# facebookresearch/wmar

Hardware: AMD Instinct MI355X
Metric: watermarked images/sec at 256x256 (16x16 tok), batch 64; detector p-value delta vs ref (higher is better)
Workload: dtype f32; 1 GPU; Taming cin_transformer (48L x 1536d x 24h, V=16384) + VQGAN f16/16384, 256x256, batch 64 per GPU, greenlist watermark delta=2 gamma=0.25 h=1 (linear/stratifiedrand), T=1 top-k 250 top-p 0.92; sample -> decode -> re-encode -> detect; random-init weights; batch_per_gpu=64, decode_loop=hipGraph replay, backend=nccl

## Files before the change

include/wmar_hip.h:

```cpp
#ifndef WMAR_HIP_H
#define WMAR_HIP_H

#include <stdint.h>

#ifdef __cplusplus
extern "C" {
#endif

#define WMAR_OK 0
#define WMAR_EINVAL (-1)
#define WMAR_EHIP (-2)
#define WMAR_ESHORT (-3)
#define WMAR_MAX_CONTEXT 16
#define WMAR_ENOMEM (-4)
#define WMAR_EMISSING (-5)
#define WMAR_ECALLBACK (-6)

#define WMAR_SEED_FIXED 0
#define WMAR_SEED_LINEAR 1
#define WMAR_SEED_SPATIAL 2
#define WMAR_SPLIT_RAND 0
#define WMAR_SPLIT_STRATIFIED 1

const char* wmar_last_error(void);
// ... 206 lines not shown
int wmar_cham_sample(const wmar_wm_ctx* wm, const float* logits3_dev, int64_t B, int64_t V, const int64_t* past_ids_dev,
                     int64_t t, int64_t past_stride, float temperature, double top_p, float guidance_scale_text,
                     float guidance_scale_image, const uint32_t* allow_dev, const int32_t* allow_ids_dev, int32_t n_allow,
                     const float* q_dev, float* scratch_dev, int64_t* tok_out_dev, void* stream);

typedef struct wmar_vq_config {
    int32_t ch, num_res_blocks, resolution, in_channels, out_ch, z_channels, embed_dim, n_embed;
    int32_t n_levels;
    int32_t ch_mult[8];
    int32_t n_attn_res;
    int32_t attn_resolutions[8];
    int32_t max_batch;
} wmar_vq_config;

typedef struct wmar_vq wmar_vq;

int wmar_vq_create(const wmar_vq_config* cfg, const char* const* names, const void* const* tensors_dev,
                   int32_t n_tensors, void* stream, wmar_vq** out);
void wmar_vq_destroy(wmar_vq* v);
int64_t wmar_vq_device_bytes(const wmar_vq* v);

int wmar_vq_decode(wmar_vq* v, const int64_t* codes_dev, int64_t B, float* images_dev, void* stream);
int wmar_vq_encode(wmar_vq* v, const float* images_dev, int64_t B, int64_t* codes_dev, float* prequant_dev,
                   void* stream);

int wmar_vq_probe_conv(const float* w_dev, const float* bias_dev, int32_t cout, int32_t cin, int32_t ks, const float* x_dev,
                       const float* res_dev, const float* gn_gamma_dev, const float* gn_beta_dev, int32_t gn_swish, int64_t B, int32_t Hs,
                       int32_t Ws, int32_t stride, int32_t up, int32_t arm_stats, float* y_dev, float* out_mr_dev, char* kernel_buf,
                       int64_t buf_len, void* stream);
int wmar_vq_probe_attn(const float* q_dev, const float* k_dev, const float* v_dev, int64_t B, int32_t H, int32_t W, int32_t C, float* o_dev,
                       char* path_buf, int64_t buf_len, void* stream);
int wmar_vq_probe_argmin(const float* z_dev, int64_t P, int32_t E, const float* codebook_dev, int32_t n_embed, int64_t* codes_dev,
                         char* path_buf, int64_t buf_len, void* stream);

int wmar_vq_probe_conv_backward(const float* w_dev, int32_t cout, int32_t cin, int32_t ks, const float* x_dev, const float* gy_dev, int64_t B,
                                int32_t Hs, int32_t Ws, int32_t stride, int32_t up, float* gx_dev, float* gw_dev, float* gb_dev,
                                char* kernel_buf, int64_t buf_len, void* stream);
int wmar_vq_probe_gn_backward(const float* x_dev, const float* gy_dev, const float* mr_dev, const float* gamma_dev, const float* beta_dev,
                              int64_t B, int32_t HW, int32_t C, int32_t swish, float* gx_dev, float* dgamma_dev, float* dbeta_dev,
                              char* path_buf, int64_t buf_len, void* stream);
int wmar_vq_probe_attn_backward(const float* q_dev, const float* k_dev, const float* v_dev, const float* go_dev, int64_t B, int32_t H, int32_t W,
                                int32_t C, float* gq_dev, float* gk_dev, float* gv_dev, char* path_buf, int64_t buf_len, void* stream);

int wmar_vq_probe_avgpool_backward(const float* gy_dev, int64_t B, int32_t Ho, int32_t Wo, int32_t C, float* gx_dev, void* stream);
int wmar_mvq_probe_image_backward(const float* pre_dev, const float* g_nchw_dev, int64_t B, int32_t C, int32_t HW, int32_t Cs, float* g_nhwc_dev,
                                  void* stream);
int wmar_mvq_probe_input_backward(const float* g_nhwc_dev, int64_t B, int32_t C, int32_t HW, int32_t Cs, float* g_nchw_dev, void* stream);

typedef struct wmar_vq_train wmar_vq_train;
int wmar_vq_train_create(const wmar_vq_config* cfg, const char* const* names, const void* const* tensors_dev, int32_t n_tensors, void* stream,
                         wmar_vq_train** out);
void wmar_vq_train_destroy(wmar_vq_train* t);
int64_t wmar_vq_train_device_bytes(const wmar_vq_train* t);
int wmar_vq_train_set_weights(wmar_vq_train* t, const char* const* names, const void* const* tensors_dev, int32_t n_tensors, void* stream);
int wmar_vq_train_encode(wmar_vq_train* t, const float* images_dev, int64_t B, float* prequant_dev, void* stream);
int wmar_vq_train_encode_backward(wmar_vq_train* t, const float* grad_prequant_dev, int64_t B, float* grad_images_dev, void* stream);
int wmar_vq_train_decode(wmar_vq_train* t, const float* zq_dev, int64_t B, float* images_dev, void* stream);
int wmar_vq_train_decode_backward(wmar_vq_train* t, const float* grad_images_dev, int64_t B, float* grad_zq_dev, void* stream);
int wmar_vq_train_get_grads(wmar_vq_train* t, const char* const* names, void* const* grads_dev, int32_t n, int32_t accumulate, void* stream);

typedef struct wmar_mvq_config {
    int32_t hidden_channels, num_res_blocks, resolution, num_channels, z_channels, num_embeddings;
    int32_t n_levels;
    int32_t channel_mult[8];
    int32_t max_batch;
} wmar_mvq_config;
// ... 61 lines not shown
```

wmar_amd/_lib.py:

```python
from __future__ import annotations

import ctypes as C
import os

HERE = os.path.dirname(os.path.abspath(__file__))
LIB_PATH = os.path.join(HERE, "libwmar_hip.so")

SYMBOLS = [
    "wmar_last_error", "wmar_version", "wmar_key_row_words", "wmar_key_table_rows", "wmar_key_table_build",
    "wmar_key_greenlist", "wmar_wm_process_logits", "wmar_sample_fused", "wmar_detect", "wmar_detect_num_ngrams",
    "wmar_gpt_create", "wmar_gpt_destroy", "wmar_gpt_device_bytes", "wmar_gpt_decode_step", "wmar_gpt_generate",
    "wmar_gpt_set_timing", "wmar_gpt_set_attention_phases", "wmar_gpt_get_timing", "wmar_gpt_profile_role", "wmar_gpt_plan_info", "wmar_gpt_check",
    "wmar_gpt_probe_run", "wmar_gpt_probe_copy", "wmar_gpt_probe_plan", "wmar_rar_create", "wmar_rar_destroy",
    "wmar_rar_device_bytes", "wmar_rar_forward_position", "wmar_rar_generate", "wmar_vq_create", "wmar_vq_destroy", "wmar_vq_device_bytes",
    "wmar_vq_decode", "wmar_vq_encode", "wmar_vq_probe_conv", "wmar_vq_probe_attn", "wmar_vq_probe_argmin", "wmar_vq_probe_conv_backward", "wmar_vq_probe_gn_backward", "wmar_vq_probe_attn_backward",
    "wmar_vq_probe_avgpool_backward", "wmar_mvq_probe_image_backward", "wmar_mvq_probe_input_backward", "wmar_mvq_train_create",
    "wmar_vq_train_create", "wmar_vq_train_destroy", "wmar_vq_train_device_bytes", "wmar_vq_train_set_weights", "wmar_vq_train_encode",
    "wmar_vq_train_encode_backward", "wmar_vq_train_decode", "wmar_vq_train_decode_backward", "wmar_vq_train_get_grads", "wmar_mvq_create", "wmar_mvq_destroy", "wmar_mvq_device_bytes", "wmar_mvq_decode",
    "wmar_mvq_encode", "wmar_gumbel_key_build", "wmar_gumbel_sample", "wmar_gumbel_score", "wmar_gumbel_key_rows", "wmar_gumbel_score_ctx", "wmar_rar_generate_gumbel", "wmar_rar_generate_gumbel_ctx", "wmar_rar_check", "wmar_rar_launch_status",
    "wmar_cham_create", "wmar_cham_destroy", "wmar_cham_device_bytes", "wmar_cham_forward_tokens", "wmar_cham_generate_image",
    "wmar_cham_sample", "wmar_cham_probe_run", "wmar_cham_probe_copy", "wmar_cham_probe_plan",
    "wmar_cfg_mix", "wmar_gpt_generate_hooked", "wmar_rar_generate_hooked", "wmar_cham_generate_image_hooked",
    "wmar_augment", "wmar_augment_backward", "wmar_jpeg_workspace_bytes", "wmar_jpeg", "wmar_resample_coeffs", "wmar_image_ingest",
    "wmar_sync_positions", "wmar_sync_workspace_bytes", "wmar_sync_fit", "wmar_sync_rotate_labels",
    "wmar_comm_unique_id", "wmar_comm_init", "wmar_comm_bcast", "wmar_comm_allgather", "wmar_comm_rank", "wmar_comm_world", "wmar_comm_destroy",
]

WMAR_ESHORT = -3
WMAR_ECALLBACK = -6

LOGITS_HOOK = C.CFUNCTYPE(C.c_int, C.c_void_p, C.c_int32, C.c_int64)


class KeyParams(C.Structure):
    _fields_ = [("salt_key", C.c_uint64), ("alive_ids", C.POINTER(C.c_int64)), ("n_alive", C.c_int64),
                ("dead_ids", C.POINTER(C.c_int64)), ("n_dead", C.c_int64), ("vocab_size", C.c_int64),
                ("gamma", C.c_double), ("split_strategy", C.c_int32), ("seed_strategy", C.c_int32)]


class WmCtx(C.Structure):
    _fields_ = [("table_dev", C.c_void_p), ("n_rows", C.c_int64), ("vocab_size", C.c_int64),
                ("seed_strategy", C.c_int32), ("context_size", C.c_int32), ("spatial_dim", C.c_int32),
                ("delta", C.c_float)]


class GptConfig(C.Structure):
    _fields_ = [("vocab_size", C.c_int32), ("block_size", C.c_int32), ("n_layer", C.c_int32),
                ("n_head", C.c_int32), ("n_embd", C.c_int32), ("max_batch", C.c_int32)]
# ... 110 lines not shown
    L.wmar_gpt_plan_info.argtypes = [vp, i64, C.c_char_p, i64]
    L.wmar_gpt_check.argtypes = [vp, vp]
    L.wmar_gpt_probe_run.argtypes = [vp, vp, i64, i32, i32, i32, i32, vp, vp]
    L.wmar_gpt_probe_copy.restype = i64
    L.wmar_gpt_probe_copy.argtypes = [vp, C.c_char_p, i32, vp, i64, i32, vp]
    L.wmar_gpt_probe_plan.argtypes = [vp, i64, i32, C.c_char_p, i64]
    L.wmar_rar_create.argtypes = [C.POINTER(RarConfig), C.POINTER(C.c_char_p), C.POINTER(vp), i32, vp, C.POINTER(vp)]
    L.wmar_rar_destroy.argtypes = [vp]
    L.wmar_rar_destroy.restype = None
    L.wmar_rar_device_bytes.restype = i64
    L.wmar_rar_device_bytes.argtypes = [vp]
    L.wmar_rar_forward_position.argtypes = [vp, vp, vp, i64, i32, vp, vp]
    L.wmar_rar_generate.argtypes = [vp, C.POINTER(WmCtx), vp, i64, C.POINTER(f32), i32, f32, vp, vp, i32, vp]
    L.wmar_rar_generate_gumbel.argtypes = [vp, vp, i64, C.POINTER(f32), i32, f32, f32, i32, vp, vp, i32, vp]
    L.wmar_rar_generate_gumbel_ctx.argtypes = [vp, vp, i64, C.POINTER(f32), i32, f32, f32, i32, C.c_uint64, i32, vp, vp, i32, vp]
    L.wmar_rar_check.argtypes = [vp, vp]
    L.wmar_rar_launch_status.argtypes = [vp, C.POINTER(i32), C.POINTER(i32)]
    L.wmar_gumbel_key_build.argtypes = [C.c_uint64, i64, vp, vp, vp]
    L.wmar_gumbel_sample.argtypes = [vp, i64, i64, vp, i64, i32, f32, f32, i32, vp, vp]
    L.wmar_gumbel_score.argtypes = [vp, i64, i64, i64, vp, i64, vp, vp, vp]
    L.wmar_gumbel_key_rows.argtypes = [vp, i64, i64, vp, vp, vp, vp]
    L.wmar_gumbel_score_ctx.argtypes = [vp, i64, i64, i64, C.c_uint64, i32, vp, vp, vp, vp]
    if hasattr(L, "wmar_vq_create"):
        L.wmar_vq_create.argtypes = [C.POINTER(VqConfig), C.POINTER(C.c_char_p), C.POINTER(vp), i32, vp, C.POINTER(vp)]
        L.wmar_vq_destroy.argtypes = [vp]
        L.wmar_vq_destroy.restype = None
        L.wmar_vq_device_bytes.restype = i64
        L.wmar_vq_device_bytes.argtypes = [vp]
        L.wmar_vq_decode.argtypes = [vp, vp, i64, vp, vp]
        L.wmar_vq_encode.argtypes = [vp, vp, i64, vp, vp, vp]
        L.wmar_vq_probe_conv.argtypes = [vp, vp, i32, i32, i32, vp, vp, vp, vp, i32, i64, i32, i32, i32, i32, i32, vp, vp, C.c_char_p, i64, vp]
        L.wmar_vq_probe_attn.argtypes = [vp, vp, vp, i64, i32, i32, i32, vp, C.c_char_p, i64, vp]
        L.wmar_vq_probe_argmin.argtypes = [vp, i64, i32, vp, i32, vp, C.c_char_p, i64, vp]
        L.wmar_vq_probe_conv_backward.argtypes = [vp, i32, i32, i32, vp, vp, i64, i32, i32, i32, i32, vp, vp, vp, C.c_char_p, i64, vp]
        L.wmar_vq_probe_gn_backward.argtypes = [vp, vp, vp, vp, vp, i64, i32, i32, i32, vp, vp, vp, C.c_char_p, i64, vp]
        L.wmar_vq_probe_attn_backward.argtypes = [vp, vp, vp, vp, i64, i32, i32, i32, vp, vp, vp, C.c_char_p, i64, vp]
        L.wmar_vq_probe_avgpool_backward.argtypes = [vp, i64, i32, i32, i32, vp, vp]
        L.wmar_mvq_probe_image_backward.argtypes = [vp, vp, i64, i32, i32, i32, vp, vp]
        L.wmar_mvq_probe_input_backward.argtypes = [vp, i64, i32, i32, i32, vp, vp]
        L.wmar_mvq_train_create.argtypes = [C.POINTER(MvqConfig), C.POINTER(C.c_char_p), C.POINTER(vp), i32, vp, C.POINTER(vp)]
        L.wmar_vq_train_create.argtypes = [C.POINTER(VqConfig), C.POINTER(C.c_char_p), C.POINTER(vp), i32, vp, C.POINTER(vp)]
        L.wmar_vq_train_destroy.argtypes = [vp]
        L.wmar_vq_train_destroy.restype = None
        L.wmar_vq_train_device_bytes.restype = i64
        L.wmar_vq_train_device_bytes.argtypes = [vp]
        L.wmar_vq_train_set_weights.argtypes = [vp, C.POINTER(C.c_char_p), C.POINTER(vp), i32, vp]
        L.wmar_vq_train_encode.argtypes = [vp, vp, i64, vp, vp]
        L.wmar_vq_train_encode_backward.argtypes = [vp, vp, i64, vp, vp]
        L.wmar_vq_train_decode.argtypes = [vp, vp, i64, vp, vp]
        L.wmar_vq_train_decode_backward.argtypes = [vp, vp, i64, vp, vp]
        L.wmar_vq_train_get_grads.argtypes = [vp, C.POINTER(C.c_char_p), C.POINTER(vp), i32, i32, vp]
    L.wmar_cham_create.argtypes = [C.POINTER(ChamConfig), C.POINTER(C.c_char_p), C.POINTER(vp), i32, vp, C.POINTER(vp)]
    L.wmar_cham_destroy.argtypes = [vp]
    L.wmar_cham_destroy.restype = None
    L.wmar_cham_device_bytes.restype = i64
    L.wmar_cham_device_bytes.argtypes = [vp]
    L.wmar_cham_forward_tokens.argtypes = [vp, vp, vp, i64, vp, vp]
    L.wmar_cham_probe_run.argtypes = [vp, vp, vp, i64, i32, i32, i32, vp, vp]
    L.wmar_cham_probe_copy.restype = i64
    L.wmar_cham_probe_copy.argtypes = [vp, C.c_char_p, i32, vp, i64, i32, vp]
    L.wmar_cham_probe_plan.argtypes = [vp, i64, C.c_char_p, i64]
    L.wmar_cham_generate_image.argtypes = [vp, C.POINTER(WmCtx), vp, vp, i64, C.POINTER(ChamSampleParams), vp, vp, i32, vp, i32, vp, vp]
    L.wmar_cham_sample.argtypes = [C.POINTER(WmCtx), vp, i64, i64, vp, i64, i64, f32, f64, f32, f32, vp, vp, i32, vp, vp, vp, vp]
    L.wmar_cfg_mix.argtypes = [vp, vp, vp, vp, i64, i64, vp, vp, f32, f32, vp]
    L.wmar_gpt_generate_hooked.argtypes = [vp, C.POINTER(SampleParams), vp, i64, i32, vp, vp, vp, vp, i64, LOGITS_HOOK, vp, vp]
    L.wmar_rar_generate_hooked.argtypes = [vp, vp, i64, C.POINTER(f32), i32, f32, vp, vp, i32, vp, vp, i64, LOGITS_HOOK, vp, vp]
# ... 33 lines not shown
```

wmar_amd/csrc/vqgan.hip:

```cpp
#include <algorithm>
#include <map>
#include <memory>
#include <string>
#include <vector>

#include "common.h"
#include "bx_split.h"
#include "vq_plan.h"

namespace wmar {

using f32x16 = __attribute__((ext_vector_type(16))) float;

__global__ void k_pack_conv(const float* __restrict__ W, float4* __restrict__ Wp, int Cout, int Cin, int ks,
                            int CT, int KBc) {
    const int T = ks * ks;
    long long idx = (long long)blockIdx.x * blockDim.x + threadIdx.x;
    long long total = (long long)CT * T * KBc * 64;
    if (idx >= total) return;
    int lane = (int)(idx & 63);
    long long r = idx >> 6;
    int kb = (int)(r % KBc); r /= KBc;
    int tap = (int)(r % T);
    int ct = (int)(r / T);
// ... 7 lines not shown
    Wp[idx] = make_float4(v[0], v[1], v[2], v[3]);
}

__global__ void k_pack_conv_bx(const float* __restrict__ W, u32x4* __restrict__ Wq, int Cout, int Cin, int ks, int CT, int KU,
                               long long w_bstride = 0, long long wq_bstride = 0, int transposed = 0) {
    const int T = ks * ks;
    const long long idx = (long long)blockIdx.x * blockDim.x + threadIdx.x;
    if (idx >= (long long)CT * T * KU * 64) return;
    W += (long long)blockIdx.y * w_bstride;
    Wq += (long long)blockIdx.y * wq_bstride;
    const int lane = (int)(idx & 63);
    long long r = idx >> 6;
    const int ku = (int)(r % KU); r /= KU;
    const int tap = (int)(r % T);
    const int ct = (int)(r / T);
    const int co = ct * 32 + (lane & 31), ci0 = ku * 16 + 8 * (lane >> 5);
    float v[8];
    for (int i = 0; i < 8; ++i)
        v[i] = (co < Cout && ci0 + i < Cin) ? (transposed ? W[(long long)(ci0 + i) * Cout + co] : W[((long long)co * Cin + ci0 + i) * T + tap]) : 0.f;
    unsigned h[4], m[4], l[4];
    for (int i = 0; i < 4; ++i) bx_split2(v[2 * i], v[2 * i + 1], h[i], m[i], l[i]);
    u32x4* o = Wq + (idx >> 6) * 192 + lane;
    o[0] = u32x4{h[0], h[1], h[2], h[3]}; o[64] = u32x4{m[0], m[1], m[2], m[3]}; o[128] = u32x4{l[0], l[1], l[2], l[3]};
}

__global__ void k_pad_vec(const float* __restrict__ src, float* __restrict__ dst, int n, int npad) {
    int i = blockIdx.x * blockDim.x + threadIdx.x;
    if (i < npad) dst[i] = i < n ? src[i] : 0.f;
}

struct ConvArgs {
    const float* in;
    const float4* wp;
    const u32x4* wq;
    long long wq_bstride;
    const float* bias;
    const float* res;
    float* out;
    int Hs, Ws, Cin;
    int Ho, Wo, Cout_s;
    int CT, KBc;
    int ks, stride, up, pad;
    int tiles_x, tiles_y;
    int dbuf;
    const float2* gn_mr;
    const float* gn_g; const float* gn_b;
    int gn_cpg, gn_swish;
    double* st_part;
    int st_cpg;
};

__device__ __forceinline__ float4 conv_gn(const ConvArgs& a, float4 v, int b, int c) {
    const float4 g = *(const float4*)(a.gn_g + c), bt = *(const float4*)(a.gn_b + c);
    float r[4] = {v.x, v.y, v.z, v.w};
    const float gg[4] = {g.x, g.y, g.z, g.w}, bb[4] = {bt.x, bt.y, bt.z, bt.w};
    const float2* mr = a.gn_mr + b * 32;
    if (a.gn_cpg >= 4 && (a.gn_cpg & 3) == 0) {
        const float2 m = mr[c / a.gn_cpg];
#pragma unroll
        for (int i = 0; i < 4; ++i) r[i] = (r[i] - m.x) * m.y * gg[i] + bb[i];
    } else {
#pragma unroll
        for (int i = 0; i < 4; ++i) { const float2 m = mr[(c + i) / a.gn_cpg]; r[i] = (r[i] - m.x) * m.y * gg[i] + bb[i]; }
    }
    if (a.gn_swish)
#pragma unroll
        for (int i = 0; i < 4; ++i) r[i] = r[i] / (1.0f + __expf(-r[i]));
    return make_float4(r[0], r[1], r[2], r[3]);
}

__device__ __forceinline__ float4 conv_gn_apply(float4 v, const float4 g, const float4 bt, const float2 m, int swish) {
    float r[4] = {(v.x - m.x) * m.y * g.x + bt.x, (v.y - m.x) * m.y * g.y + bt.y, (v.z - m.x) * m.y * g.z + bt.z, (v.w - m.x) * m.y * g.w + bt.w};
    if (swish)
#pragma unroll
        for (int i = 0; i < 4; ++i) r[i] = r[i] / (1.0f + __expf(-r[i]));
    return make_float4(r[0], r[1], r[2], r[3]);
}

__device__ __forceinline__ void conv_store(const ConvArgs& a, const f32x16 (&acc)[2], int b, int ct, int ty, int tx, int lane) {
    const int j = lane & 31, half = lane >> 5;
    const int prow = j >> 3, pcol = j & 7;
    const int oy0 = ty * 8, ox0 = tx * 8;
    double gs[4] = {0.0, 0.0, 0.0, 0.0}, gss[4] = {0.0, 0.0, 0.0, 0.0};
#pragma unroll
    for (int p = 0; p < 2; ++p) {
        const int oy = oy0 + p * 4 + prow, ox = ox0 + pcol;
        const long long pix = ((long long)b * a.Ho + oy) * a.Wo + ox;
#pragma unroll
        for (int g = 0; g < 4; ++g) {
            const int co = ct * 32 + g * 8 + half * 4;
            if (co >= a.Cout_s) continue;
            const float4 bb = *(const float4*)(a.bias + co);
            float4 o = make_float4(acc[p][g * 4 + 0] + bb.x, acc[p][g * 4 + 1] + bb.y, acc[p][g * 4 + 2] + bb.z,
                                   acc[p][g * 4 + 3] + bb.w);
            if (a.res) {
                const float4 rr = *(const float4*)(a.res + pix * a.Cout_s + co);
                o.x += rr.x; o.y += rr.y; o.z += rr.z; o.w += rr.w;
            }
            *(float4*)(a.out + pix * a.Cout_s + co) = o;
            if (a.st_part) {
                gs[g] += (double)o.x + (double)o.y + (double)o.z + (double)o.w;
                gss[g] += sq4_f64(o);
            }
        }
    }
    if (a.st_part) {
        const int top = a.st_cpg >= 8 ? 32 : 16;
#pragma unroll
        for (int g = 0; g < 4; ++g)
            for (int o = 1; o <= top; o <<= 1) { gs[g] += __shfl_xor(gs[g], o); gss[g] += __shfl_xor(gss[g], o); }
        if (a.st_cpg == 16) { gs[0] += gs[1]; gss[0] += gss[1]; gs[2] += gs[3]; gss[2] += gss[3]; }
        const long long tile = ((long long)b * a.tiles_y + ty) * a.tiles_x + tx;
        double* dst = a.st_part + tile * 64;
        if (a.st_cpg == 4) {
            if ((lane & 31) == 0)
#pragma unroll
                for (int g = 0; g < 4; ++g) { const int grp = ct * 8 + 2 * g + half; dst[grp * 2] = gs[g]; dst[grp * 2 + 1] = gss[g]; }
        } else if (lane == 0) {
            if (a.st_cpg == 8) {
#pragma unroll
                for (int g = 0; g < 4; ++g) { const int grp = ct * 4 + g; dst[grp * 2] = gs[g]; dst[grp * 2 + 1] = gss[g]; }
            } else {
                dst[(ct * 2) * 2] = gs[0]; dst[(ct * 2) * 2 + 1] = gss[0];
                dst[(ct * 2 + 1) * 2] = gs[2]; dst[(ct * 2 + 1) * 2 + 1] = gss[2];
            }
        }
    }
}

constexpr int CONV_CCH = 32;
constexpr int CONV_PSTRIDE = 36;

template <int COT>
__global__ __launch_bounds__(COT * 64) void k_conv(ConvArgs a) {
    extern __shared__ __attribute__((aligned(16))) float patch[];
    const int lane = threadIdx.x & 63;
    const int w = __builtin_amdgcn_readfirstlane(threadIdx.x >> 6);
    int bid = blockIdx.x;
    const int tx = bid % a.tiles_x; bid /= a.tiles_x;
    const int ty = bid % a.tiles_y; bid /= a.tiles_y;
    const int cgroups = (a.CT + COT - 1) / COT;
    const int cg = bid % cgroups;
    const int b = bid / cgroups;
    const int ct = cg * COT + w;
    const bool active = ct < a.CT;
    const int T = a.ks * a.ks;
    const int PW = 7 * a.stride + a.ks, PH = PW;
    const int oy0 = ty * 8, ox0 = tx * 8;
    const int iy0 = oy0 * a.stride - a.pad, ix0 = ox0 * a.stride - a.pad;
    const int Hc = a.up ? a.Hs * 2 : a.Hs, Wc = a.up ? a.Ws * 2 : a.Ws;

    f32x16 acc[2];
#pragma unroll
    for (int i = 0; i < 2; ++i)
#pragma unroll
        for (int r = 0; r < 16; ++r) acc[i][r] = 0.f;

    const int j = lane & 31, half = lane >> 5;
    const int prow = j >> 3, pcol = j & 7;
    const float* inb = a.in + (long long)b * a.Hs * a.Ws * a.Cin;

#define WMAR_CONV_ROUND(PATCH, C0, CCH)                                                                         \
    if (active) {                                                                                               \
        const int nkb = (CCH) >> 3;                                                                             \
        const float4* wbase = a.wp + ((long long)ct * T * a.KBc + ((C0) >> 3)) * 64 + lane;                     \
        for (int tap = 0; tap < T; ++tap) {                                                                     \
            const int dy = tap / a.ks, dx = tap - dy * a.ks;                                                    \
            const float4* wt = wbase + (long long)tap * a.KBc * 64;                                             \
            const float* p0 = (PATCH) + (((prow)*a.stride + dy) * PW + pcol * a.stride + dx) * CONV_PSTRIDE + half * 4; \
            const float* p1 = p0 + 4 * a.stride * PW * CONV_PSTRIDE;                                            \
            _Pragma("unroll 4") for (int kb = 0; kb < nkb; ++kb) {                                              \
                const float4 wv = wt[kb * 64];                                                                  \
                const float4 x0 = *(const float4*)(p0 + kb * 8);                                                \
                const float4 x1 = *(const float4*)(p1 + kb * 8);                                                \
                acc[0] = __builtin_amdgcn_mfma_f32_32x32x2f32(wv.x, x0.x, acc[0], 0, 0, 0);                     \
                acc[1] = __builtin_amdgcn_mfma_f32_32x32x2f32(wv.x, x1.x, acc[1], 0, 0, 0);                     \
// ... 348 lines not shown
    if (threadIdx.x < 32) { acc[threadIdx.x][0] = 0; acc[threadIdx.x][1] = 0; }
    __syncthreads();
    __shared__ double tmp[256][4][2];
    for (int i = 0; i < 4; ++i) { tmp[threadIdx.x][i][0] = s[i]; tmp[threadIdx.x][i][1] = ss[i]; }
    __syncthreads();
    if (threadIdx.x < 32) {
        const int g = threadIdx.x;
        double ts = 0, tss = 0;
        for (int t = 0; t < 256; ++t) {
            if (t / q4 >= pstep) break;
            const int c = (t % q4) * 4;
            for (int i = 0; i < 4; ++i)
                if ((c + i) / cpg == g) { ts += tmp[t][i][0]; tss += tmp[t][i][1]; }
        }
        double* o = a.partial + (((long long)b * a.nchunk + chunk) * 32 + g) * 2;
        o[0] = ts; o[1] = tss;
    }
}

__global__ void k_gn_finalize(GnArgs a, float2* mr) {
    const int b = blockIdx.x, g = threadIdx.x;
    double ts = 0, tss = 0;
    for (int c = 0; c < a.nchunk; ++c) {
        const double* p = a.partial + (((long long)b * a.nchunk + c) * 32 + g) * 2;
        ts += p[0]; tss += p[1];
    }
    const double n = (double)a.HW * (a.C / 32);
    const double rn = inv_count_f64(n);
    const double mean = ts * rn;
    const double var = var_f64(tss * rn, mean);
    mr[b * 32 + g] = make_float2((float)mean, (float)rsqrt_f64(var + 1e-6));
}

__global__ __launch_bounds__(256) void k_gn_finalize_tiles(const double* part, int tiles, double count, float2* mr) {
    __shared__ double red[8][32][2];
    const int b = blockIdx.x, g = threadIdx.x & 31, q = threadIdx.x >> 5;
    const double* p = part + (long long)b * tiles * 64 + g * 2;
    double ts = 0, tss = 0;
    for (int t = q; t < tiles; t += 8) { ts += p[(long long)t * 64]; tss += p[(long long)t * 64 + 1]; }
    red[q][g][0] = ts; red[q][g][1] = tss;
    __syncthreads();
    if (threadIdx.x < 32) {
        ts = 0; tss = 0;
        for (int i = 0; i < 8; ++i) { ts += red[i][g][0]; tss += red[i][g][1]; }
        const double rn = inv_count_f64(count);
        const double mean = ts * rn;
        const double var = var_f64(tss * rn, mean);
        mr[b * 32 + g] = make_float2((float)mean, (float)rsqrt_f64(var + 1e-6));
    }
}

__global__ __launch_bounds__(256) void k_attn_scores(const float* __restrict__ q, const float* __restrict__ k,
                                                     float* __restrict__ sc, int N, int C, float scale) {
    extern __shared__ float qs[];
    __shared__ float red[4];
    const int b = blockIdx.y, i = blockIdx.x;
    const float* qi = q + ((long long)b * N + i) * C;
    for (int c = threadIdx.x; c < C; c += 256) qs[c] = qi[c];
    __syncthreads();
    float* row = sc + ((long long)b * N + i) * N;
    float mx = -INFINITY;
    for (int j = threadIdx.x; j < N; j += 256) {
        const float* kj = k + ((long long)b * N + j) * C;
        float s = 0.f;
        for (int c = 0; c < C; c += 4) {
            float4 kv = *(const float4*)(kj + c);
            s += qs[c] * kv.x + qs[c + 1] * kv.y + qs[c + 2] * kv.z + qs[c + 3] * kv.w;
        }
        s *= scale;
        row[j] = s;
        mx = fmaxf(mx, s);
    }
    for (int o = 32; o > 0; o >>= 1) mx = fmaxf(mx, __shfl_xor(mx, o));
    if ((threadIdx.x & 63) == 0) red[threadIdx.x >> 6] = mx;
    __syncthreads();
    mx = fmaxf(fmaxf(red[0], red[1]), fmaxf(red[2], red[3]));
    __syncthreads();
// ... 349 lines not shown
static thread_local int g_vq_splits = 0;

struct GnRef {
    const float2* mr; const float* g; const float* b; int C, swish;
};

int run_conv(const ConvW& c, const float* in, float* out, const float* res, int B, int Hs, int Ws, int stride, int up,
             hipStream_t st, const GnRef* gn = nullptr, long long wq_bstride = 0) {
    ConvArgs a{};
    if (gn) {
        WMAR_REQUIRE(gn->C == c.cin_s && !up, "fused GroupNorm: channel count %d != conv input %d", gn->C, c.cin_s);
        a.gn_mr = gn->mr; a.gn_g = gn->g; a.gn_b = gn->b; a.gn_cpg = gn->C / 32; a.gn_swish = gn->swish;
    }
    a.in = in; a.wp = c.wp; a.wq = c.wq; a.wq_bstride = wq_bstride; a.bias = c.bias; a.res = res; a.out = out;
    a.Hs = Hs; a.Ws = Ws; a.Cin = c.cin_s;
    const int Hc = up ? 2 * Hs : Hs, Wc = up ? 2 * Ws : Ws;
    a.Ho = stride == 2 ? Hc / 2 : Hc; a.Wo = stride == 2 ? Wc / 2 : Wc;
    a.Cout_s = c.cout_s; a.CT = c.CT; a.KBc = c.KBc; a.ks = c.ks; a.stride = stride; a.up = up;
    a.pad = (c.ks == 3 && stride == 1) ? 1 : 0;
    WMAR_REQUIRE(a.Ho % 8 == 0 && a.Wo % 8 == 0, "conv output %dx%d is not a multiple of the 8x8 tile", a.Ho, a.Wo);
    a.tiles_x = a.Wo / 8; a.tiles_y = a.Ho / 8;
    const int PW = 7 * stride + c.ks;
    const int COT = c.CT >= 4 ? 4 : (c.CT >= 2 ? 2 : 1);
    a.dbuf = (c.cin_s % CONV_CCH == 0 && PW * PW * 8 <= 4 * COT * 64) ? 1 : 0;
    const int cpg_out = c.cout / 32;
    const bool stats = wq_bstride == 0 && g_trk.part && c.cout == c.cout_s && c.cout % 32 == 0 && (cpg_out == 4 || cpg_out == 8 || cpg_out == 16) &&
                       (long long)B * a.tiles_x * a.tiles_y * 64 <= g_trk.cap;
    if (stats) { a.st_part = g_trk.part; a.st_cpg = cpg_out; g_trk.src = out; g_trk.tiles = a.tiles_x * a.tiles_y; g_trk.C = c.cout; }
    else if (g_trk.src == out) g_trk.src = nullptr;
    const bool bx2 = c.wq && c.cin_s % CONV_CCH == 0 && stride == 2 && c.ks == 3 && COT == 4 && !up && !conv_no_bx() && conv_s2_bx();
    const bool bx = (c.wq && c.cin_s % CONV_CCH == 0 && stride == 1 && (c.ks == 3 || c.ks == 1) && !conv_no_bx()) || bx2;
    if (bx) a.dbuf = 1;
    const bool wide = bx && !bx2 && COT == 4 && c.ks == 3 && a.tiles_x % 2 == 0 && wq_bstride == 0 && conv_pt4();
    const size_t lds = bx ? (size_t)2 * PW * (wide ? PW + 8 : PW) * CONV_PSTRIDE_BX : (size_t)(a.dbuf ? 2 : 1) * PW * PW * CONV_PSTRIDE * sizeof(float);
    const int cgroups = (c.CT + COT - 1) / COT;
    const unsigned grid = (unsigned)((long long)B * cgroups * (wide ? a.tiles_x / 2 : a.tiles_x) * a.tiles_y);
    hipEvent_t e0 = nullptr, e1 = nullptr;
    if (vq_trace()) { (void)hipEventCreate(&e0); (void)hipEventCreate(&e1); (void)hipEventRecord(e0, st); }
    static const bool few_off = getenv("WMAR_CONV_FEW_OFF") != nullptr;
    const bool few = c.wf && c.ks == 3 && stride == 1 && !up && !res && !stats && wq_bstride == 0 && c.cout <= 4 && a.Ho % CF_T == 0 &&
                     a.Wo % CF_T == 0 && !few_off;
    if (few) {
        a.tiles_x = a.Wo / CF_T; a.tiles_y = a.Ho / CF_T;
        const unsigned gridf = (unsigned)((long long)B * a.tiles_x * a.tiles_y);
        const size_t ldsf = (size_t)CF_PW * CF_PW * CONV_PSTRIDE * sizeof(float);
        if (c.cout == 3) { g_conv_kernel = "k_conv_few<3>"; hipLaunchKernelGGL(k_conv_few<3>, dim3(gridf), dim3(256), ldsf, st, a, (const float*)c.wf); }
        else { g_conv_kernel = "k_conv_few<4>"; hipLaunchKernelGGL(k_conv_few<4>, dim3(gridf), dim3(256), ldsf, st, a, (const float*)c.wf); }
    } else if (bx2) {
        static const hipError_t lds2_ok = hipFuncSetAttribute((const void*)k_conv_bx<4, 3, 2, 2>, hipFuncAttributeMaxDynamicSharedMemorySize, 160 * 1024);
        WMAR_REQUIRE(lds2_ok == hipSuccess, "k_conv_bx (stride 2): raising the dynamic LDS limit failed: %s", hipGetErrorString(lds2_ok));
        g_conv_kernel = "k_conv_bx<4,3,2,2>";
        hipLaunchKernelGGL((k_conv_bx<4, 3, 2, 2>), dim3(grid), dim3(256), lds, st, a);
    } else if (wide) {
        static const hipError_t lds_ok = hipFuncSetAttribute((const void*)k_conv_bx<4, 3, 4>, hipFuncAttributeMaxDynamicSharedMemorySize, 160 * 1024);
        WMAR_REQUIRE(lds_ok == hipSuccess, "k_conv_bx: raising the dynamic LDS limit failed: %s", hipGetErrorString(lds_ok));
        g_conv_kernel = "k_conv_bx<4,3,4>";
        hipLaunchKernelGGL((k_conv_bx<4, 3, 4>), dim3(grid), dim3(256), lds, st, a);
    }
    else if (bx && COT == 4 && c.ks == 3) { g_conv_kernel = "k_conv_bx<4,3>"; hipLaunchKernelGGL((k_conv_bx<4, 3>), dim3(grid), dim3(256), lds, st, a); }
    else if (bx && COT == 4) { g_conv_kernel = "k_conv_bx<4,1>"; hipLaunchKernelGGL((k_conv_bx<4, 1>), dim3(grid), dim3(256), lds, st, a); }
    else if (bx && COT == 2 && c.ks == 3) { g_conv_kernel = "k_conv_bx<2,3>"; hipLaunchKernelGGL((k_conv_bx<2, 3>), dim3(grid), dim3(128), lds, st, a); }
    else if (bx && COT == 2) { g_conv_kernel = "k_conv_bx<2,1>"; hipLaunchKernelGGL((k_conv_bx<2, 1>), dim3(grid), dim3(128), lds, st, a); }
    else if (bx && c.ks == 3) { g_conv_kernel = "k_conv_bx<1,3>"; hipLaunchKernelGGL((k_conv_bx<1, 3>), dim3(grid), dim3(64), lds, st, a); }
    else if (bx) { g_conv_kernel = "k_conv_bx<1,1>"; hipLaunchKernelGGL((k_conv_bx<1, 1>), dim3(grid), dim3(64), lds, st, a); }
    else if (COT == 4) { g_conv_kernel = "k_conv<4>"; hipLaunchKernelGGL(k_conv<4>, dim3(grid), dim3(256), lds, st, a); }
    else if (COT == 2) { g_conv_kernel = "k_conv<2>"; hipLaunchKernelGGL(k_conv<2>, dim3(grid), dim3(128), lds, st, a); }
    else { g_conv_kernel = "k_conv<1>"; hipLaunchKernelGGL(k_conv<1>, dim3(grid), dim3(64), lds, st, a); }
// ... 13 lines not shown
    const int KB = a.E >> 3, NT = a.n_embed >> 5;
    const size_t lds4 = (size_t)128 * (a.E + 4) * sizeof(float);
    if (!split_off && best && a.P >= 128 && KB % 8 == 0 && NT >= 4 && lds4 <= 150 * 1024) {
        const long long groups = (a.P + 127) / 128;
        int CS = 1;
        while (groups * CS * 2 <= 256 && NT % (CS * 2) == 0 && NT / (CS * 2) >= 4) CS *= 2;
        WMAR_HIP_CHECK(hipMemsetAsync(best, 0xff, (size_t)a.P * 8, st));
        static const hipError_t lds_ok = hipFuncSetAttribute((const void*)k_vq_argmin_split<4>, hipFuncAttributeMaxDynamicSharedMemorySize, 152 * 1024);
        WMAR_REQUIRE(lds_ok == hipSuccess, "k_vq_argmin_split: raising the dynamic LDS limit failed: %s", hipGetErrorString(lds_ok));
        g_vq_splits = CS;
        hipLaunchKernelGGL(k_vq_argmin_split<4>, dim3((unsigned)(groups * CS)), dim3(256), lds4, st, a, best, CS);
        hipLaunchKernelGGL(k_vq_finish, dim3((unsigned)((a.P + 255) / 256)), dim3(256), 0, st, (const unsigned long long*)best, a.codes, a.P);
        return launch_status("k_vq_argmin_split");
    }
    const size_t lds = (size_t)64 * (a.E + 4) * sizeof(float);
    WMAR_HIP_CHECK(hipFuncSetAttribute((const void*)k_vq_argmin, hipFuncAttributeMaxDynamicSharedMemorySize, (int)lds));
    g_vq_splits = 0;
    hipLaunchKernelGGL(k_vq_argmin, dim3((unsigned)((a.P + 63) / 64)), dim3(256), lds, st, a);
    return launch_status("k_vq_argmin");
}

int run_gn(double* gn_partial, const NormW& n, const float* x, int B, int HW, int swish, hipStream_t st, GnRef* out) {
    GnArgs a{};
    a.x = x; a.y = nullptr; a.partial = gn_partial + GN_MR_DOUBLES; a.gamma = n.g; a.beta = n.b; a.HW = HW; a.C = n.C; a.swish = swish;
    WMAR_REQUIRE(n.C % 32 == 0 && n.C / 4 <= 256, "GroupNorm channel count %d unsupported (multiple of 32, <= 1024)", n.C);
    int nchunk = HW / 256;
    if (nchunk < 1) nchunk = 1;
    if (nchunk > GN_CHUNKS_MAX) nchunk = GN_CHUNKS_MAX;
    a.nchunk = nchunk;
    WMAR_REQUIRE(B <= GN_MR_DOUBLES / 32, "GroupNorm: batch %d too large", B);
    float2* mr = (float2*)gn_partial;
    if (g_trk.part && g_trk.src == x && g_trk.C == n.C && g_trk.tiles * 64 == HW) {
        g_gn_path = "k_gn_finalize_tiles";
        hipLaunchKernelGGL(k_gn_finalize_tiles, dim3(B), dim3(256), 0, st, (const double*)g_trk.part, g_trk.tiles,
                           (double)HW * (n.C / 32), mr);
    } else {
        g_gn_path = "k_gn_partial+k_gn_finalize";
        hipLaunchKernelGGL(k_gn_partial, dim3(nchunk, B), dim3(256), 0, st, a);
        hipLaunchKernelGGL(k_gn_finalize, dim3(B), dim3(32), 0, st, a, mr);
    }
    out->mr = mr; out->g = n.g; out->b = n.b; out->C = n.C; out->swish = swish;
    return launch_status("k_gn");
}

struct AttnScratch { float* asc; u32x4* attk; u32x4* attv; float* zbias; };
static thread_local const char *g_attn_path = "none", *g_attn_scores = "none", *g_attn_pv = "none";

int attn_core(const AttnScratch& s, const float* q, const float* k, const float* vv, float* o, int B, int H, int W, int C, hipStream_t st) {
    int rc;
    const int N = H * W;
    const float scale = 1.0f / sqrtf((float)C);
    if (s.attk && N % 32 == 0 && C % 32 == 0 && H % 8 == 0 && W % 8 == 0 && N >= 64 && C >= 64 && !conv_no_bx()) {
        ConvW ck{}, cv{};
        ck.wq = s.attk; ck.bias = s.zbias; ck.cin = ck.cin_s = C; ck.cout = ck.cout_s = N; ck.ks = 1; ck.CT = N / 32; ck.KBc = C / 8;
        cv.wq = s.attv; cv.bias = s.zbias; cv.cin = cv.cin_s = N; cv.cout = cv.cout_s = C; cv.ks = 1; cv.CT = C / 32; cv.KBc = N / 8;
        const long long sk = (long long)ck.CT * (C / 16) * 192, sv = (long long)cv.CT * (N / 16) * 192;
        const long long nk = (long long)ck.CT * (C / 16) * 64, nv = (long long)cv.CT * (N / 16) * 64;
        hipLaunchKernelGGL(k_pack_conv_bx, dim3((unsigned)((nk + 255) / 256), B), dim3(256), 0, st, k, s.attk, N, C, 1, ck.CT,
                           C / 16, (long long)N * C, sk, 0);
        hipLaunchKernelGGL(k_pack_conv_bx, dim3((unsigned)((nv + 255) / 256), B), dim3(256), 0, st, vv, s.attv, C, N, 1, cv.CT,
                           N / 16, (long long)N * C, sv, 1);
        if ((rc = launch_status("k_pack_conv_bx"))) return rc;
        if ((rc = run_conv(ck, q, s.asc, nullptr, B, H, W, 1, 0, st, nullptr, sk))) return rc;
        g_attn_scores = g_conv_kernel;
        hipLaunchKernelGGL(k_attn_softmax, dim3((unsigned)(((long long)B * N + 3) / 4)), dim3(256), 0, st, s.asc, (long long)B * N, N, scale);
        if ((rc = launch_status("k_attn_softmax"))) return rc;
        if ((rc = run_conv(cv, s.asc, o, nullptr, B, H, W, 1, 0, st, nullptr, sv))) return rc;
        g_attn_path = "bf16_pipe"; g_attn_pv = g_conv_kernel;
// ... 112 lines not shown
        const int n = snprintf(path_buf, (size_t)buf_len, "path=%s;scores=%s;pv=%s", g_attn_path, g_attn_scores, g_attn_pv);
        if (!(n > 0 && n < buf_len)) { set_error("vq_probe_attn: buffer of %lld bytes too small", (long long)buf_len); rc = WMAR_EINVAL; }
    }
    return probe_finish(rc, st);
}

int wmar_vq_probe_argmin(const float* z_dev, int64_t P, int32_t E, const float* codebook_dev, int32_t n_embed, int64_t* codes_dev,
                         char* path_buf, int64_t buf_len, void* stream) {
    WMAR_REQUIRE(z_dev && codebook_dev && codes_dev && path_buf && buf_len > 0, "vq_probe_argmin: null argument");
    WMAR_REQUIRE(P >= 1 && E >= 8 && E % 8 == 0 && n_embed >= 32 && n_embed % 32 == 0, "vq_probe_argmin: embed_dim %% 8 and n_embed %% 32 must be 0");
    hipStream_t st = (hipStream_t)stream;
    DeviceArena mem;
    float4* emb_p = nullptr; float *enorm = nullptr, *znorm = nullptr; unsigned long long* best = nullptr;
    int rc = WMAR_OK;
    WMAR_TRY(mem.alloc(&emb_p, (size_t)n_embed * E / 4));
    WMAR_TRY(mem.alloc(&enorm, (size_t)n_embed));
    WMAR_TRY(mem.alloc(&znorm, (size_t)P));
    WMAR_TRY(mem.alloc(&best, (size_t)P));
    WMAR_TRY(pack_codebook(codebook_dev, emb_p, enorm, n_embed, E, st));
    if (rc == WMAR_OK) {
        hipLaunchKernelGGL(k_row_sqnorm, dim3((unsigned)P), dim3(64), 0, st, z_dev, znorm, E);
        VqArgs a{};
        a.z = z_dev; a.ep = emb_p; a.enorm = enorm; a.znorm = znorm; a.codes = (long long*)codes_dev; a.P = P; a.E = E; a.n_embed = n_embed;
        rc = run_vq_argmin(a, best, st);
    }
    if (rc == WMAR_OK) {
        const int n = g_vq_splits > 0 ? snprintf(path_buf, (size_t)buf_len, "k_vq_argmin_split<4> (%d code splits)", g_vq_splits)
                                      : snprintf(path_buf, (size_t)buf_len, "k_vq_argmin");
        if (!(n > 0 && n < buf_len)) { set_error("vq_probe_argmin: buffer of %lld bytes too small", (long long)buf_len); rc = WMAR_EINVAL; }
    }
    return probe_finish(rc, st);
}

}

namespace wmar {

__global__ void k_avgpool2(const float* __restrict__ in, float* __restrict__ out, int Ho, int Wo, int C) {
    const long long q4 = C >> 2;
    const long long total = (long long)Ho * Wo * q4;
    const long long b = blockIdx.y;
    const float* ib = in + b * (long long)(2 * Ho) * (2 * Wo) * C;
    float* ob = out + b * (long long)Ho * Wo * C;
    for (long long e = (long long)blockIdx.x * blockDim.x + threadIdx.x; e < total; e += (long long)gridDim.x * blockDim.x) {
        const int c = (int)(e % q4) * 4;
        const long long pix = e / q4;
        const int ox = (int)(pix % Wo), oy = (int)(pix / Wo);
        const float* p = ib + ((long long)(2 * oy) * (2 * Wo) + 2 * ox) * C + c;
        const float4 a = *(const float4*)p, b2 = *(const float4*)(p + C);
        const float4 c2 = *(const float4*)(p + (long long)2 * Wo * C), d = *(const float4*)(p + (long long)2 * Wo * C + C);
        *(float4*)(ob + pix * C + c) = make_float4((a.x + b2.x + c2.x + d.x) / 4.0f, (a.y + b2.y + c2.y + d.y) / 4.0f,
                                                   (a.z + b2.z + c2.z + d.z) / 4.0f, (a.w + b2.w + c2.w + d.w) / 4.0f);
    }
}

__global__ void k_nchw_to_nhwc01(const float* __restrict__ src, float* __restrict__ dst, int C, int HW, int Cs) {
    long long idx = (long long)blockIdx.x * blockDim.x + threadIdx.x;
    const long long b = blockIdx.y;
    if (idx >= HW) return;
    for (int c = 0; c < Cs; ++c)
        dst[((long long)b * HW + idx) * Cs + c] = c < C ? (src[((long long)b * C + c) * HW + idx] + 1.0f) / 2.0f : 0.f;
}

__global__ void k_nhwc_to_nchw_01(const float* __restrict__ src, float* __restrict__ dst, int C, int HW, int Cs) {
    long long idx = (long long)blockIdx.x * blockDim.x + threadIdx.x;
    const long long b = blockIdx.y;
// ... 219 lines not shown
```

Baseline: 59.99 images/s.

## Add a specialised 3-channel conv path and parallelise GroupNorm tile finalize

Adds a conv_k27 path for 3x3 stride-1 convolutions with 3 input channels, such as the encoder's first conv on RGB images. It treats the 27 taps as a K dimension for MFMA, stages the input patch in LDS, and writes output through an LDS staging buffer so global stores are coalesced. This replaces the generic path, which is wasteful when Cin is tiny. It also splits the GroupNorm finalize-from-tiles kernel across 4x more blocks with vectorised double2 loads and shuffle reductions, and adds a probe entry point. The new conv path adds LDS use and an env switch to disable it.

```diff
diff --git a/include/wmar_hip.h b/include/wmar_hip.h
--- a/include/wmar_hip.h
+++ b/include/wmar_hip.h
@@ -262,6 +262,7 @@
                        char* path_buf, int64_t buf_len, void* stream);
 int wmar_vq_probe_argmin(const float* z_dev, int64_t P, int32_t E, const float* codebook_dev, int32_t n_embed, int64_t* codes_dev,
                          char* path_buf, int64_t buf_len, void* stream);
+int wmar_vq_probe_gn_tiles(const double* part_dev, int64_t B, int32_t tiles, double count, double* sums_dev, float* mr_dev, void* stream);
 
 int wmar_vq_probe_conv_backward(const float* w_dev, int32_t cout, int32_t cin, int32_t ks, const float* x_dev, const float* gy_dev, int64_t B,
                                 int32_t Hs, int32_t Ws, int32_t stride, int32_t up, float* gx_dev, float* gw_dev, float* gb_dev,
diff --git a/wmar_amd/_lib.py b/wmar_amd/_lib.py
--- a/wmar_amd/_lib.py
+++ b/wmar_amd/_lib.py
@@ -13,7 +13,7 @@
     "wmar_gpt_set_timing", "wmar_gpt_set_attention_phases", "wmar_gpt_get_timing", "wmar_gpt_profile_role", "wmar_gpt_plan_info", "wmar_gpt_check",
     "wmar_gpt_probe_run", "wmar_gpt_probe_copy", "wmar_gpt_probe_plan", "wmar_rar_create", "wmar_rar_destroy",
     "wmar_rar_device_bytes", "wmar_rar_forward_position", "wmar_rar_generate", "wmar_vq_create", "wmar_vq_destroy", "wmar_vq_device_bytes",
-    "wmar_vq_decode", "wmar_vq_encode", "wmar_vq_probe_conv", "wmar_vq_probe_attn", "wmar_vq_probe_argmin", "wmar_vq_probe_conv_backward", "wmar_vq_probe_gn_backward", "wmar_vq_probe_attn_backward",
+    "wmar_vq_decode", "wmar_vq_encode", "wmar_vq_probe_conv", "wmar_vq_probe_attn", "wmar_vq_probe_argmin", "wmar_vq_probe_gn_tiles", "wmar_vq_probe_conv_backward", "wmar_vq_probe_gn_backward", "wmar_vq_probe_attn_backward",
     "wmar_vq_probe_avgpool_backward", "wmar_mvq_probe_image_backward", "wmar_mvq_probe_input_backward", "wmar_mvq_train_create",
     "wmar_vq_train_create", "wmar_vq_train_destroy", "wmar_vq_train_device_bytes", "wmar_vq_train_set_weights", "wmar_vq_train_encode",
     "wmar_vq_train_encode_backward", "wmar_vq_train_decode", "wmar_vq_train_decode_backward", "wmar_vq_train_get_grads", "wmar_mvq_create", "wmar_mvq_destroy", "wmar_mvq_device_bytes", "wmar_mvq_decode",
@@ -190,6 +190,7 @@
         L.wmar_vq_probe_conv.argtypes = [vp, vp, i32, i32, i32, vp, vp, vp, vp, i32, i64, i32, i32, i32, i32, i32, vp, vp, C.c_char_p, i64, vp]
         L.wmar_vq_probe_attn.argtypes = [vp, vp, vp, i64, i32, i32, i32, vp, C.c_char_p, i64, vp]
         L.wmar_vq_probe_argmin.argtypes = [vp, i64, i32, vp, i32, vp, C.c_char_p, i64, vp]
+        L.wmar_vq_probe_gn_tiles.argtypes = [vp, i64, i32, C.c_double, vp, vp, vp]
         L.wmar_vq_probe_conv_backward.argtypes = [vp, i32, i32, i32, vp, vp, i64, i32, i32, i32, i32, vp, vp, vp, C.c_char_p, i64, vp]
         L.wmar_vq_probe_gn_backward.argtypes = [vp, vp, vp, vp, vp, i64, i32, i32, i32, vp, vp, vp, C.c_char_p, i64, vp]
         L.wmar_vq_probe_attn_backward.argtypes = [vp, vp, vp, vp, i64, i32, i32, i32, vp, vp, vp, C.c_char_p, i64, vp]
diff --git a/wmar_amd/csrc/vqgan.hip b/wmar_amd/csrc/vqgan.hip
--- a/wmar_amd/csrc/vqgan.hip
+++ b/wmar_amd/csrc/vqgan.hip
@@ -63,6 +63,7 @@
 struct ConvArgs {
     const float* in;
     const float4* wp;
+    int k27;
     const u32x4* wq;
     long long wq_bstride;
     const float* bias;
@@ -108,7 +109,8 @@
     return make_float4(r[0], r[1], r[2], r[3]);
 }
 
-__device__ __forceinline__ void conv_store(const ConvArgs& a, const f32x16 (&acc)[2], int b, int ct, int ty, int tx, int lane) {
+__device__ __forceinline__ void conv_store(const ConvArgs& a, const f32x16 (&acc)[2], int b, int ct, int ty, int tx, int lane,
+                                           float* stage = nullptr, int sstride = 0, int sco = 0) {
     const int j = lane & 31, half = lane >> 5;
     const int prow = j >> 3, pcol = j & 7;
     const int oy0 = ty * 8, ox0 = tx * 8;
@@ -128,7 +130,8 @@
                 const float4 rr = *(const float4*)(a.res + pix * a.Cout_s + co);
                 o.x += rr.x; o.y += rr.y; o.z += rr.z; o.w += rr.w;
             }
-            *(float4*)(a.out + pix * a.Cout_s + co) = o;
+            if (stage) *(float4*)(stage + (p * 32 + j) * sstride + sco + g * 8 + half * 4) = o;
+            else *(float4*)(a.out + pix * a.Cout_s + co) = o;
             if (a.st_part) {
                 gs[g] += (double)o.x + (double)o.y + (double)o.z + (double)o.w;
                 gss[g] += sq4_f64(o);
@@ -161,6 +164,61 @@
 
 constexpr int CONV_CCH = 32;
 constexpr int CONV_PSTRIDE = 36;
+
+constexpr int CK_STEPS = 14;
+constexpr int CK_PP = 112;
+constexpr int ck_ostride(int cot) { return cot * 32 + 4; }
+constexpr size_t ck_lds_bytes(int cot) { return (size_t)(3 * CK_PP + 64 * ck_ostride(cot)) * sizeof(float); }
+
+template <int COT>
+__device__ __forceinline__ void conv_k27(const ConvArgs& a, float* lds, int b, int cg, int ty, int tx, int w, int lane) {
+    float* pat = lds;
+    float* stage = lds + 3 * CK_PP;
+    constexpr int OS = ck_ostride(COT);
+    const int ct = cg * COT + w;
+    const int oy0 = ty * 8, ox0 = tx * 8;
+    const float* inb = a.in + (long long)b * a.Hs * a.Ws * a.Cin;
+    for (int e = threadIdx.x; e < 100; e += COT * 64) {
+        const int py = e / 10, px = e - py * 10;
+        const int y = oy0 - 1 + py, x = ox0 - 1 + px;
+        float4 v = make_float4(0.f, 0.f, 0.f, 0.f);
+        if (y >= 0 && y < a.Hs && x >= 0 && x < a.Ws) v = *(const float4*)(inb + ((long long)y * a.Ws + x) * a.Cin);
+        pat[e] = v.x; pat[CK_PP + e] = v.y; pat[2 * CK_PP + e] = v.z;
+    }
+    const float* wrow = (const float*)(a.wp + (long long)ct * 9 * a.KBc * 64 + (lane & 31));
+    float wv[CK_STEPS];
+#pragma unroll
+    for (int s = 0; s < CK_STEPS; ++s) {
+        const int k0 = 2 * s, k1 = 2 * s + 1 < 27 ? 2 * s + 1 : 26;
+        const float* wp_ = wrow + ((lane >> 5) ? (k1 / 3) * a.KBc * 256 + k1 % 3 : (k0 / 3) * a.KBc * 256 + k0 % 3);
+        wv[s] = *wp_;
+    }
+    if (lane >> 5) wv[CK_STEPS - 1] = 0.f;
+    __syncthreads();
+    f32x16 acc[2];
+#pragma unroll
+    for (int i = 0; i < 2; ++i)
+#pragma unroll
+        for (int r = 0; r < 16; ++r) acc[i][r] = 0.f;
+    const int j = lane & 31, half = lane >> 5;
+    const float* p0 = pat + (j >> 3) * 10 + (j & 7);
+#pragma unroll
+    for (int s = 0; s < CK_STEPS; ++s) {
+        const int k0 = 2 * s, k1 = 2 * s + 1 < 27 ? 2 * s + 1 : 26;
+        const int o0 = (k0 % 3) * CK_PP + (k0 / 9) * 10 + (k0 / 3) % 3, o1 = (k1 % 3) * CK_PP + (k1 / 9) * 10 + (k1 / 3) % 3;
+        const float* px = p0 + (half ? o1 : o0);
+        acc[0] = __builtin_amdgcn_mfma_f32_32x32x2f32(wv[s], px[0], acc[0], 0, 0, 0);
+        acc[1] = __builtin_amdgcn_mfma_f32_32x32x2f32(wv[s], px[40], acc[1], 0, 0, 0);
+    }
+    conv_store(a, acc, b, ct, ty, tx, lane, stage, OS, w * 32);
+    __syncthreads();
+    constexpr int Q = COT * 8;
+    for (int e = threadIdx.x; e < 64 * Q; e += COT * 64) {
+        const int pix = e / Q, q = e - pix * Q;
+        const long long gp = ((long long)b * a.Ho + oy0 + (pix >> 3)) * a.Wo + ox0 + (pix & 7);
+        *(float4*)(a.out + gp * a.Cout_s + cg * (COT * 32) + q * 4) = *(const float4*)(stage + pix * OS + q * 4);
+    }
+}
 
 template <int COT>
 __global__ __launch_bounds__(COT * 64) void k_conv(ConvArgs a) {
@@ -173,6 +231,7 @@
     const int cgroups = (a.CT + COT - 1) / COT;
     const int cg = bid % cgroups;
     const int b = bid / cgroups;
+    if (a.k27) { conv_k27<COT>(a, patch, b, cg, ty, tx, w, lane); return; }
     const int ct = cg * COT + w;
     const bool active = ct < a.CT;
     const int T = a.ks * a.ks;
@@ -587,17 +646,34 @@
     mr[b * 32 + g] = make_float2((float)mean, (float)rsqrt_f64(var + 1e-6));
 }
 
-__global__ __launch_bounds__(256) void k_gn_finalize_tiles(const double* part, int tiles, double count, float2* mr) {
-    __shared__ double red[8][32][2];
-    const int b = blockIdx.x, g = threadIdx.x & 31, q = threadIdx.x >> 5;
-    const double* p = part + (long long)b * tiles * 64 + g * 2;
-    double ts = 0, tss = 0;
-    for (int t = q; t < tiles; t += 8) { ts += p[(long long)t * 64]; tss += p[(long long)t * 64 + 1]; }
-    red[q][g][0] = ts; red[q][g][1] = tss;
+__device__ __forceinline__ double gn_tree8(const double (&v)[8]) { return ((v[0] + v[1]) + (v[2] + v[3])) + ((v[4] + v[5]) + (v[6] + v[7])); }
+
+__global__ __launch_bounds__(256) void k_gn_finalize_tiles(const double* __restrict__ part, int tiles, double count, float2* __restrict__ mr,
+                                                           double* __restrict__ sums) {
+    __shared__ double red[4][8][2];
+    const int b = blockIdx.x >> 2, g = (blockIdx.x & 3) * 8 + (threadIdx.x & 7), q = threadIdx.x >> 3;
+    const double2* p = (const double2*)(part + (long long)b * tiles * 64) + g;
+    double s[8], ss[8];
+#pragma unroll
+    for (int i = 0; i < 8; ++i) { s[i] = 0.0; ss[i] = 0.0; }
+    for (int t0 = q; t0 < tiles; t0 += 256) {
+        double2 v[8];
+#pragma unroll
+        for (int i = 0; i < 8; ++i) v[i] = p[(long long)min(t0 + 32 * i, tiles - 1) * 32];
+        __builtin_amdgcn_sched_barrier(0);
+#pragma unroll
+        for (int i = 0; i < 8; ++i) { const bool in = t0 + 32 * i < tiles; s[i] += in ? v[i].x : 0.0; ss[i] += in ? v[i].y : 0.0; }
+    }
+    double ts = gn_tree8(s), tss = gn_tree8(ss);
+#pragma unroll
+    for (int o = 8; o <= 32; o <<= 1) { ts += __shfl_xor(ts, o); tss += __shfl_xor(tss, o); }
+    if ((threadIdx.x & 63) < 8) { red[threadIdx.x >> 6][threadIdx.x & 7][0] = ts; red[threadIdx.x >> 6][threadIdx.x & 7][1] = tss; }
     __syncthreads();
-    if (threadIdx.x < 32) {
-        ts = 0; tss = 0;
-        for (int i = 0; i < 8; ++i) { ts += red[i][g][0]; tss += red[i][g][1]; }
+    if (threadIdx.x < 8) {
+        const int l = threadIdx.x;
+        ts = (red[0][l][0] + red[1][l][0]) + (red[2][l][0] + red[3][l][0]);
+        tss = (red[0][l][1] + red[1][l][1]) + (red[2][l][1] + red[3][l][1]);
+        if (sums) { sums[(b * 32 + g) * 2] = ts; sums[(b * 32 + g) * 2 + 1] = tss; }
         const double rn = inv_count_f64(count);
         const double mean = ts * rn;
         const double var = var_f64(tss * rn, mean);
@@ -1013,7 +1089,12 @@
     const bool bx = (c.wq && c.cin_s % CONV_CCH == 0 && stride == 1 && (c.ks == 3 || c.ks == 1) && !conv_no_bx()) || bx2;
     if (bx) a.dbuf = 1;
     const bool wide = bx && !bx2 && COT == 4 && c.ks == 3 && a.tiles_x % 2 == 0 && wq_bstride == 0 && conv_pt4();
-    const size_t lds = bx ? (size_t)2 * PW * (wide ? PW + 8 : PW) * CONV_PSTRIDE_BX : (size_t)(a.dbuf ? 2 : 1) * PW * PW * CONV_PSTRIDE * sizeof(float);
+    static const bool k27_off = getenv("WMAR_CONV_K27_OFF") != nullptr;
+    const bool k27 = !bx && c.wp && c.ks == 3 && c.cin == 3 && stride == 1 && !up && !gn && wq_bstride == 0 && c.CT % COT == 0 &&
+                     c.cout_s == c.CT * 32 && !k27_off;
+    a.k27 = k27 ? 1 : 0;
+    const size_t lds = bx ? (size_t)2 * PW * (wide ? PW + 8 : PW) * CONV_PSTRIDE_BX
+                     : k27 ? ck_lds_bytes(COT) : (size_t)(a.dbuf ? 2 : 1) * PW * PW * CONV_PSTRIDE * sizeof(float);
     const int cgroups = (c.CT + COT - 1) / COT;
     const unsigned grid = (unsigned)((long long)B * cgroups * (wide ? a.tiles_x / 2 : a.tiles_x) * a.tiles_y);
     hipEvent_t e0 = nullptr, e1 = nullptr;
@@ -1093,8 +1174,8 @@
     float2* mr = (float2*)gn_partial;
     if (g_trk.part && g_trk.src == x && g_trk.C == n.C && g_trk.tiles * 64 == HW) {
         g_gn_path = "k_gn_finalize_tiles";
-        hipLaunchKernelGGL(k_gn_finalize_tiles, dim3(B), dim3(256), 0, st, (const double*)g_trk.part, g_trk.tiles,
-                           (double)HW * (n.C / 32), mr);
+        hipLaunchKernelGGL(k_gn_finalize_tiles, dim3(B * 4), dim3(256), 0, st, (const double*)g_trk.part, g_trk.tiles,
+                           (double)HW * (n.C / 32), mr, (double*)nullptr);
     } else {
         g_gn_path = "k_gn_partial+k_gn_finalize";
         hipLaunchKernelGGL(k_gn_partial, dim3(nchunk, B), dim3(256), 0, st, a);
@@ -1273,6 +1354,14 @@
     return probe_finish(rc, st);
 }
 
+int wmar_vq_probe_gn_tiles(const double* part_dev, int64_t B, int32_t tiles, double count, double* sums_dev, float* mr_dev, void* stream) {
+    WMAR_REQUIRE(part_dev && mr_dev, "vq_probe_gn_tiles: null argument");
+    WMAR_REQUIRE(B >= 1 && B <= 1024 && tiles >= 1 && count > 0, "vq_probe_gn_tiles: bad shape");
+    hipStream_t st = (hipStream_t)stream;
+    hipLaunchKernelGGL(k_gn_finalize_tiles, dim3((unsigned)B * 4), dim3(256), 0, st, part_dev, (int)tiles, count, (float2*)mr_dev, sums_dev);
+    return probe_finish(launch_status("k_gn_finalize_tiles"), st);
+}
+
 }
 
 namespace wmar {
```

Result: no change. 60.06 images/s, median of 6 (+0.1%).
